# ghazalehnt/RecBole

Measured on AMD Instinct MI355X. Metric: train positives/sec (+neg) per node, higher is better.
Workload: dtype fp32; 1 GPU; C2 BPR-MF ml-20m-shape: 138,494 users x 26,745 items (incl. PAD), ~20M interactions RO_RS 0.8/0.1/0.1, embedding 128, 4 uniform negatives, 512 positives (2,048 rows) per step, dense Adam; global_batch=512, per_gpu_batch=512, train_interactions=16014928, parallelism=single, exchange_graph=True, sampler=walk (bit-exact)

## Files before the change

### include/mirec.h

```cpp
#ifndef MIREC_H
#define MIREC_H

#include <stddef.h>
#include <stdint.h>

#ifdef __cplusplus
extern "C" {
#endif

#define MIREC_ABI_VERSION 18

int mirec_abi_version(void);
const char* mirec_last_error(void);

size_t mirec_sample_walk_workspace_size(int64_t batch_keys, int64_t num);
int mirec_sample_walk(const int32_t* random_list, int64_t L, int64_t* pr_dev,
                      const int64_t* keys, int64_t n_keys, int64_t batch_keys,
                      int64_t n_batches, int64_t num,
                      const int64_t* used_ptr, const int32_t* used_cols,
                      const uint32_t* used_bits, int64_t n_bits,
                      int64_t n_key_space, int reject,
                      int64_t* out, int64_t out_stride, int32_t* status_dev,
                      void* ws, size_t ws_bytes, void* stream);

int mirec_sample_walk_segments(const int32_t* random_list, int64_t L, int64_t* pr_dev,
// ... 211 lines not shown
                            int32_t step_off, double beta1, double beta2, double eps,
                            double weight_decay, void* stream);
int mirec_adam_deferred_pair_f32(const mirec_adam_table* tables, const int64_t* n_max_uniq,
                                 int32_t d, const float* step_consts_dev,
                                 const int32_t* step_base_dev, int32_t step_off, double beta1,
                                 double beta2, double eps, double weight_decay, void* stream);

int mirec_adam_flush_f32(const mirec_adam_table* tables, int32_t n_tables, int32_t d,
                         const float* step_consts_dev, const int32_t* step_base_dev,
                         int32_t step_off, double beta1, double beta2, double eps,
                         double weight_decay, void* stream);
int mirec_adam_flush_rows_f32(const mirec_adam_table* tables, int32_t n_tables, int32_t d,
                              const int32_t* rows_per_wave, const float* step_consts_dev,
                              const int32_t* step_base_dev, int32_t step_off, double beta1,
                              double beta2, double eps, double weight_decay, void* stream);
int mirec_bpr_adam_step_f32(const mirec_adam_table* tables, const int64_t* n_max_uniq,
                            int32_t d, const int64_t* items, int64_t Bc, int32_t T, float gamma,
                            float grad_scale, float* loss_k, const int32_t* u_rec,
                            const int32_t* u_crec, const int32_t* i_rec, const int32_t* i_crec,
                            float* u_part, int32_t* u_join, float* i_part, int32_t* i_join,
                            const float* step_consts_dev, const int32_t* step_base_dev,
                            int32_t step_off, double beta1, double beta2, double eps,
                            double weight_decay, void* stream);
int mirec_step_records(const int64_t* user_keys, const int64_t* item_keys, int64_t n_batches,
                       int64_t Bc, int32_t T, int64_t n_users, int64_t n_items,
                       const int32_t* u_perm, const int32_t* u_uniq, const int32_t* u_seg,
                       const int32_t* u_nu, const int32_t* i_perm, const int32_t* i_uniq,
                       const int32_t* i_seg, const int32_t* i_nu, int32_t* u_rec,
                       int32_t* u_crec, int32_t* i_rec, int32_t* i_crec, int32_t* u_ahead,
                       int32_t* u_nah, int32_t* i_ahead, int32_t* i_nah, void* stream);
// ... 261 lines not shown
```

### recbole_amd/_native.py

```python
from __future__ import annotations

import ctypes
import os
from ctypes import c_double, c_float, c_int, c_int32, c_int64, c_size_t, c_void_p, c_char_p

import torch

_HERE = os.path.dirname(os.path.abspath(__file__))
LIB_PATH = os.environ.get("MIREC_LIB", os.path.join(_HERE, "_lib", "libmirec.so"))

_P = c_void_p


class RowsRef(ctypes.Structure):
    _fields_ = [('lo', _P), ('hi', _P), ('split', c_int64)]


class SpmmEpilogue(ctypes.Structure):
    _fields_ = [('add', RowsRef), ('add_scale', c_float), ('y', RowsRef), ('acc_in', RowsRef),
                ('acc_out', RowsRef), ('acc_scale', c_float)]


class CtxField(ctypes.Structure):
    _fields_ = [('kind', c_int32), ('seq_len', c_int32), ('ids', _P), ('vals', _P),
# ... 152 lines not shown
    "mirec_adam_flat_f32": (c_int, [_P, _P, _P, c_int64, _P, _P, _P, c_double, c_double,
                                    c_double, c_double, _P]),
    "mirec_adam_multi_f32": (c_int, [ctypes.POINTER(AdamTable), c_int32, c_int32, _P, _P,
                                     c_int32, c_double, c_double, c_double, c_double, _P]),
    "mirec_adam_deferred_f32": (c_int, [ctypes.POINTER(AdamTable), c_int32, _P, c_int32, _P,
                                        _P, c_int32, c_double, c_double, c_double, c_double,
                                        _P]),
    "mirec_adam_deferred_pair_f32": (c_int, [ctypes.POINTER(AdamTable), _P, c_int32, _P, _P,
                                             c_int32, c_double, c_double, c_double, c_double,
                                             _P]),
    "mirec_adam_flush_f32": (c_int, [ctypes.POINTER(AdamTable), c_int32, c_int32, _P, _P,
                                     c_int32, c_double, c_double, c_double, c_double, _P]),
    "mirec_adam_flush_rows_f32": (c_int, [ctypes.POINTER(AdamTable), c_int32, c_int32, _P, _P,
                                          _P, c_int32, c_double, c_double, c_double, c_double,
                                          _P]),
    "mirec_bpr_adam_step_f32": (c_int, [ctypes.POINTER(AdamTable), _P, c_int32, _P, c_int64,
                                        c_int32, ctypes.c_float, ctypes.c_float, _P, _P, _P,
                                        _P, _P, _P, _P, _P, _P, _P, _P, c_int32, c_double,
                                        c_double, c_double, c_double, _P]),
    "mirec_step_record_ints": (c_int64, [c_int64]),
    "mirec_colsum_multi_f32": (c_int, [_P, _P, _P, _P, c_int32, _P]),
    "mirec_offset_keys": (c_int, [_P, _P, c_int32, c_int64, _P, _P]),
    "mirec_bpr_fwd_bwd_at_ids_f32": (c_int, [_P, c_int64, c_int32, _P, _P, _P, c_int64, c_int32,
                                             ctypes.c_float, ctypes.c_float, _P, _P, _P]),
    "mirec_chunk_group_fits": (c_int, [c_int64, c_int32, c_int64, c_int64, c_int32]),
    "mirec_chunk_group": (c_int, [_P, _P, c_int64, c_int64, c_int32, c_int64, c_int64] + [_P] * 16
                          + [_P]),
    "mirec_step_records": (c_int, [_P, _P, c_int64, c_int64, c_int32, c_int64, c_int64, _P, _P,
                                   _P, _P, _P, _P, _P, _P, _P, _P, _P, _P, _P, _P, _P, _P,
                                   _P]),
# ... 46 lines not shown
    "mirec_seq_embed_ln_drop_fwd_f32": (c_int, [_P, c_int64, _P, _P, c_int64, c_int32, c_int32,
                                                _P, _P, c_float, c_float, ctypes.c_uint64, _P,
                                                _P, _P, _P, _P, _P]),
    "mirec_seq_embed_ln_drop_bwd_f32": (c_int, [_P, c_int64, _P, _P, c_int64, c_int32, c_int32,
                                                _P, _P, _P, _P, c_float, ctypes.c_uint64, _P,
                                                _P, _P, _P, _P, _P, _P]),
    "mirec_scale_by_f32": (c_int, [_P, c_int64, _P, _P]),
    "mirec_sampled_softmax_f32": (c_int, [_P, _P, c_int64, c_int32, _P, _P, c_int64, c_int32,
                                          c_float, _P, _P, _P, _P]),
    "mirec_rank_of_pos_f32": (c_int, [_P, _P, c_int64, c_int32, _P, _P, c_int64, c_int32, _P,
                                      _P]),
    "mirec_gather_sqnorm_f32": (c_int, [_P, c_int64, c_int32, _P, c_int64, _P, _P]),
    "mirec_gather_scale_rows_f32": (c_int, [_P, c_int64, c_int32, _P, c_int64, _P, _P, _P]),
}

ABI_VERSION = 18


class NativeError(RuntimeError):
    pass


_lib = None


def lib():
    global _lib
    if _lib is not None:
        return _lib
    if not os.path.exists(LIB_PATH):
        raise NativeError(
# ... 32 lines not shown
```

### recbole_amd/csrc/adam.hip

```cpp

#include "adam_core.h"

namespace mirec {

template <int D>
__global__ __launch_bounds__(kAdamThreads) void adam_multi_kernel(
    const AdamTables tabs, const float* __restrict__ consts, const int32_t* __restrict__ step_base,
    int step_off, AdamConsts k) {
  constexpr int VPR = D / 4;
  constexpr int RPP = kAdamThreads / VPR;
  static_assert(kAdamThreads % VPR == 0, "row width");
  __shared__ int32_t slot[kAdamRows];
  __shared__ int32_t s_range[2];

  const int si = segment_of(tabs, blockIdx.x);
  const mirec_adam_table& T = tabs.t[si];
  float* __restrict__ P = T.p;
  float* __restrict__ M = T.m;
  float* __restrict__ V = T.v;
  const int32_t* __restrict__ uniq = T.uniq;

  const int64_t lo = ((int64_t)blockIdx.x - tabs.block_start[si]) * kAdamRows;
  const int64_t hi = min(T.n_rows, lo + kAdamRows);
  if (threadIdx.x < kAdamRows) slot[threadIdx.x] = -1;
// ... 145 lines not shown
    }
  }
}

template <int D>
struct FlushVec { using T = float; };
template <> struct FlushVec<128> { using T = float2; };
template <> struct FlushVec<256> { using T = float4; };

#ifndef MIREC_FLUSH_THREADS
#define MIREC_FLUSH_THREADS 64
#endif
constexpr int kFlushRowThreads = MIREC_FLUSH_THREADS;

template <int D>
__global__ __launch_bounds__(kFlushRowThreads) void adam_flush_row_kernel(
    const AdamTables tabs, const float* __restrict__ consts, const int32_t* __restrict__ step_base,
    int step_off, AdamConsts k) {
  using V = typename FlushVec<D>::T;
  constexpr int RPB = kFlushRowThreads / 64;
  const int si = segment_of(tabs, blockIdx.x);
  const mirec_adam_table& T = tabs.t[si];
  const int64_t r = ((int64_t)blockIdx.x - tabs.block_start[si]) * RPB + (threadIdx.x >> 6);
  if (r >= T.n_rows) return;
  const int target = step_base[0] + step_off;
  const int raw = __builtin_amdgcn_readfirstlane(T.last[r]);
  const int last = min(raw, target);
  const int64_t off = r * 64 + (threadIdx.x & 63);
  const bool par = T.p_alt != nullptr;
  const bool odd = par && (target & 1);
  if (last >= target) {
    if (odd && raw != kZeroState)
      reinterpret_cast<V*>(T.p)[off] = reinterpret_cast<const V*>(T.p_alt)[off];
    return;
  }
  V p = reinterpret_cast<const V*>((par && (last & 1)) ? T.p_alt : T.p)[off];
  V m = reinterpret_cast<const V*>(T.m)[off];
  V v = reinterpret_cast<const V*>(T.v)[off];
  replay<V, true>(p, m, v, last, target, consts, k);
  MIREC_WORK(10, 1);
  if (odd) reinterpret_cast<V*>(T.p_alt)[off] = p;
  reinterpret_cast<V*>(T.p)[off] = p;
  reinterpret_cast<V*>(T.m)[off] = m;
  reinterpret_cast<V*>(T.v)[off] = v;
  if ((threadIdx.x & 63) == 0) T.last[r] = target;
}

struct FlushRows {
  int32_t r[kMaxTables];
};

template <int D>
__global__ __launch_bounds__(kAdamThreads) void adam_flush_scan_kernel(
    const AdamTables tabs, const float* __restrict__ consts, const int32_t* __restrict__ step_base,
    int step_off, AdamConsts k, FlushRows rows_per_wave) {
  using V = typename FlushVec<D>::T;
  const int si = segment_of(tabs, blockIdx.x);
  const mirec_adam_table& T = tabs.t[si];
  const int R = rows_per_wave.r[si];
  const int lane = threadIdx.x & 63;
  const int64_t r0 =
      (((int64_t)blockIdx.x - tabs.block_start[si]) * (kAdamThreads / 64) + (threadIdx.x >> 6)) * R;
  if (r0 >= T.n_rows) return;
  const int target = step_base[0] + step_off;
  const bool par = T.p_alt != nullptr;
  const bool odd = par && (target & 1);
  int raw = kZeroState;
  if (lane < R && r0 + lane < T.n_rows) raw = T.last[r0 + lane];
  const bool need = min(raw, target) < target || (odd && raw != kZeroState);
  uint64_t todo = __ballot(need);
  while (todo) {
    const int i = __builtin_ctzll(todo);
    todo &= todo - 1;
    const int64_t r = r0 + i;
    const int rraw = __shfl(raw, i, 64);
    const int last = min(rraw, target);
    const int64_t off = r * 64 + lane;
    if (last >= target) {
      reinterpret_cast<V*>(T.p)[off] = reinterpret_cast<const V*>(T.p_alt)[off];
      continue;
    }
    V p = reinterpret_cast<const V*>((par && (last & 1)) ? T.p_alt : T.p)[off];
    V m = reinterpret_cast<const V*>(T.m)[off];
    V v = reinterpret_cast<const V*>(T.v)[off];
    replay<V, true>(p, m, v, last, target, consts, k);
    MIREC_WORK(10, 1);
    if (odd) reinterpret_cast<V*>(T.p_alt)[off] = p;
    reinterpret_cast<V*>(T.p)[off] = p;
    reinterpret_cast<V*>(T.m)[off] = m;
    reinterpret_cast<V*>(T.v)[off] = v;
    if (lane == 0) T.last[r] = target;
  }
}

}

using namespace mirec;

namespace {

enum class Sched { kStreamed, kDeferred, kFlush, kDeferredPair };

int launch_adam(Sched sched, const mirec_adam_table* tables, int32_t n_tables,
                const int64_t* n_max_uniq, int32_t d, const float* consts,
                const int32_t* step_base, int32_t step_off, double beta1, double beta2,
                double eps, double weight_decay, void* stream, const char* what,
                const int32_t* flush_rows = nullptr) {
  if (n_tables < 1 || n_tables > kMaxTables || !tables || !consts || !step_base) {
    set_error("%s: bad arguments (n_tables=%d)", what, n_tables);
    return -1;
  }
  if (((uintptr_t)consts & 15) != 0) {
    set_error("%s: step constants must be 16-byte aligned", what);
    return -1;
  }
  if (d != 4 && d != 16 && d != 32 && d != 64 && d != 128 && d != 256 &&
      !(d == 1 && sched != Sched::kStreamed)) {
    set_error("%s: row width %d not in {4,16,32,64,128,256} (1: deferred / flush)", what, d);
    return -1;
  }
  const int VPR = d / 4;
  const bool pair = sched == Sched::kDeferredPair;
// ... 10 lines not shown
  for (int q = 0; q < kMaxTables; ++q) fr.r[q] = 1;
  if (sched == Sched::kFlush && flush_rows) {
    if (d < 64) {
      set_error("%s: rows per wave need d >= 64", what);
      return -1;
    }
    for (int q = 0; q < n_tables; ++q) {
      if (flush_rows[q] < 1 || flush_rows[q] > 64) {
        set_error("%s: rows per wave %d of table %d not in [1, 64]", what, flush_rows[q], q);
        return -1;
      }
      fr.r[q] = flush_rows[q];
    }
    scan = true;
  }
  AdamTables tabs;
  memset(&tabs, 0, sizeof(tabs));
  const bool deferred = sched == Sched::kDeferred;
  tabs.n_seg = deferred ? 2 * n_tables : n_tables;
  int dvec = 1;
  if (deferred && n_max_uniq && d >= 4) {
    int64_t waves = 0;
    for (int q = 0; q < (pair ? 1 : n_tables); ++q)
      if (n_max_uniq[q] > 0)
        waves += n_max_uniq[q] * (tables[q].ahead_uniq ? 2 : 1) * ((d + 63) / 64);
    if (waves > 16 * 1024) dvec = 2;
    bool ahead = false;
    for (int q = 0; q < n_tables; ++q) ahead = ahead || tables[q].ahead_uniq != nullptr;
    if (dvec == 2 && d >= 128 && !ahead && !pair) dvec = 4;
  }
// ... 3 lines not shown
    const bool grouped = t.n_uniq != nullptr;
    if (!t.p || !t.m || !t.v || t.n_rows < 0 ||
        (grouped && (!t.uniq || !t.seg || !t.perm || !t.rows)) ||
        (sched != Sched::kStreamed && !t.last) ||
        (deferred && (!grouped || t.dense_grad || !n_max_uniq || n_max_uniq[q] < 0)) ||
        (deferred && (t.ahead_uniq == nullptr) != (t.ahead_n_uniq == nullptr))) {
      set_error("%s: bad table %d", what, q);
      return -1;
    }
    if (t.p_alt && (sched == Sched::kStreamed || d < 64 || pair)) {
      set_error("%s: table %d: parity buffer (p_alt) needs the deferred schedule and d >= 64",
                what, q);
      return -1;
    }
    tabs.t[q] = t;
    if (deferred) {
      const int rpb = (pair && q == 1) ? deferred_block(1) : deferred_block(d / dvec) / (d / dvec);
      const int64_t nb = (n_max_uniq[q] + rpb - 1) / rpb;
      tabs.block_start[2 * q] = blocks;
      blocks += nb;
      tabs.block_start[2 * q + 1] = blocks;
      if (t.ahead_uniq) blocks += nb;
    } else {
      tabs.block_start[q] = blocks;
      const int64_t rows_per_block =
          scan ? (int64_t)(kAdamThreads / 64) * fr.r[q]
          : (sched == Sched::kFlush && d >= 64) ? kFlushRowThreads / 64
          : sched == Sched::kFlush ? kFlushRows
                                   : kAdamRows;
      blocks += (t.n_rows + rows_per_block - 1) / rows_per_block;
    }
// ... 15 lines not shown
  case DD:                                                                                   \
    if (sched == Sched::kStreamed)                                                           \
      hipLaunchKernelGGL(adam_multi_kernel<DD>, grd, blk, 0, st, tabs, consts, step_base,    \
                         step_off, k);                                                       \
    else if (deferred && pair)                                                               \
      hipLaunchKernelGGL((dvec == 2 ? adam_deferred_pair_kernel<DD, float2>                  \
                                    : adam_deferred_pair_kernel<DD, float>),                 \
                         grd, dim3(deferred_block(1)), 0, st, tabs, consts, step_base,       \
                         step_off, k);                                                       \
    else if (deferred)                                                                       \
      hipLaunchKernelGGL((dvec == 4 ? adam_deferred_kernel<DD, float4>                       \
                          : dvec == 2 ? adam_deferred_kernel<DD, float2>                     \
                                      : adam_deferred_kernel<DD, float>),                    \
                         grd, dim3(deferred_block(DD / dvec)), 0, st, tabs, consts,          \
                         step_base, step_off, k);                                            \
    else if (DD >= 64 && scan)                                                               \
      hipLaunchKernelGGL(adam_flush_scan_kernel<(DD >= 64 ? DD : 64)>, grd, blk, 0, st, tabs,  \
                         consts, step_base, step_off, k, fr);                                \
    else if (DD >= 64)                                                                       \
      hipLaunchKernelGGL(adam_flush_row_kernel<(DD >= 64 ? DD : 64)>, grd,                   \
                         dim3(kFlushRowThreads), 0, st, tabs,                                \
                         consts, step_base, step_off, k);                                    \
    else                                                                                     \
      hipLaunchKernelGGL(adam_flush_list_kernel<(DD < 64 ? DD : 16)>, grd, blk, 0, st, tabs, \
                         consts, step_base, step_off, k);                                    \
    break;
  switch (d) {
    case 1:
      if (deferred)
        hipLaunchKernelGGL((adam_deferred_kernel<1, float>), grd, dim3(deferred_block(1)), 0, st,
                           tabs, consts, step_base, step_off, k);
      else
        hipLaunchKernelGGL(adam_flush_list_kernel<1>, grd, blk, 0, st, tabs, consts, step_base,
// ... 66 lines not shown
extern "C" int mirec_adam_flush_rows_f32(const mirec_adam_table* tables, int32_t n_tables,
                                         int32_t d, const int32_t* rows_per_wave,
                                         const float* step_consts_dev,
                                         const int32_t* step_base_dev, int32_t step_off,
                                         double beta1, double beta2, double eps,
                                         double weight_decay, void* stream) {
  if (!rows_per_wave) {
    set_error("mirec_adam_flush_rows_f32: rows_per_wave is NULL");
    return -1;
  }
  return launch_adam(Sched::kFlush, tables, n_tables, nullptr, d, step_consts_dev,
                     step_base_dev, step_off, beta1, beta2, eps, weight_decay, stream,
                     "mirec_adam_flush_rows_f32", rows_per_wave);
}

extern "C" int mirec_adam_sparse_grad_f32(float* p, float* m, float* v, int64_t n_rows,
                                          int32_t d, const float* rows, const int32_t* perm,
                                          const int32_t* uniq, const int32_t* seg,
                                          const int32_t* n_uniq_dev, int64_t n_max_uniq,
                                          const float* dense_grad, const float* step_consts_dev,
                                          const int32_t* step_idx_dev, double beta1,
                                          double beta2, double eps, double weight_decay,
                                          void* stream) {
  (void)n_max_uniq;
  if (n_rows == 0) return 0;
  mirec_adam_table t;
  memset(&t, 0, sizeof(t));
  t.p = p; t.m = m; t.v = v; t.n_rows = n_rows;
  t.rows = rows; t.perm = perm; t.uniq = uniq; t.seg = seg; t.n_uniq = n_uniq_dev;
  t.dense_grad = dense_grad;
// ... 152 lines not shown
```

### recbole_amd/csrc/step.hip

```cpp
#include "adam_core.h"
#include "bpr_math.h"
#include "ahead.h"

namespace mirec {

struct StepLaunch {
  mirec_adam_table t[2];
  const int32_t* rec[2];
  const int32_t* crec[2];
  float* part[2];
  int32_t* join[2];
  int64_t block_start[7];
  int32_t seg_rows[6];
};

__device__ __forceinline__ int64_t clamp_id(int64_t id, int64_t n) {
  return id < 0 ? 0 : (id >= n ? n - 1 : id);
}


constexpr int kRecInts = 8;
constexpr int kRecInline = 2;
constexpr int kRowRec = 4 + kRecInline * kRecInts;
constexpr int kShare = kRecInline;
// ... 359 lines not shown
}

template <int D> struct StepVec { using T = float2; };
template <> struct StepVec<64> { using T = float; };
#ifndef MIREC_STEP_RPB
#define MIREC_STEP_RPB 4
#endif
template <int D> struct StepRows { static constexpr int n = D <= 128 ? MIREC_STEP_RPB : 1; };
#ifndef MIREC_STEP_SUM_LOADS
#define MIREC_STEP_SUM_LOADS 8
#endif
constexpr int kSumLoads = MIREC_STEP_SUM_LOADS;
#ifndef MIREC_STEP_WAVES
#define MIREC_STEP_WAVES 5
#endif

template <int D>
__global__ __launch_bounds__(D / Lanes<typename StepVec<D>::T>::n * StepRows<D>::n,
                             MIREC_STEP_WAVES)
void bpr_adam_step_kernel(
    const StepLaunch L, const int64_t* __restrict__ items, int Bc, int T, float gamma,
    float grad_scale, float* __restrict__ loss_k, const float* __restrict__ consts,
    const int32_t* __restrict__ step_base, int step_off, AdamConsts k) {
  using V = typename StepVec<D>::T;
  constexpr int EPT = Lanes<V>::n;
  constexpr int TPB = D / EPT;
  constexpr int RPB = StepRows<D>::n;
  static_assert(RPB == 1 || TPB == 64, "several rows per workgroup need one wave per row");
  constexpr int LPR = D / 4;
  constexpr int NG = TPB / LPR;
  __shared__ float cont_all[RPB][NG][D];
  __shared__ int s_last_all[RPB];
  const int wv = RPB > 1 ? __builtin_amdgcn_readfirstlane((int)(threadIdx.x / TPB)) : 0;
  auto& cont = cont_all[wv];
  int& s_last = s_last_all[wv];
  auto row_sync = [&]() {
    if (RPB == 1) {
      __syncthreads();
    } else {
      __builtin_amdgcn_fence(__ATOMIC_RELEASE, "wavefront");
      __builtin_amdgcn_wave_barrier();
      __builtin_amdgcn_fence(__ATOMIC_ACQUIRE, "wavefront");
    }
  };
  int si = 0;
// ... 250 lines not shown
    return -1;
  }
  if (n_batches == 0 || Bc == 0) return 0;
  const RecJob U = {u_perm, u_uniq, u_seg, u_nu, u_rec, u_crec, u_ahead, u_nah};
  const RecJob I = {i_perm, i_uniq, i_seg, i_nu, i_rec, i_crec, i_ahead, i_nah};
  const int64_t KI = (1 + T) * Bc;
  const int PC = (int)((KI + kPrepThreads - 1) / kPrepThreads);
  hipLaunchKernelGGL(step_prep_kernel, dim3((unsigned)(4 * n_batches + 2 * n_batches * PC)),
                     dim3(kPrepThreads), 0, (hipStream_t)stream, user_keys, item_keys,
                     (int)n_batches, (int)Bc, T, n_users, n_items, U, I, PC);
  return launch_status("mirec_step_records");
}

extern "C" int64_t mirec_step_record_ints(int64_t per) { return per < 0 ? -1 : rec_ints(per); }

#if defined(MIREC_STEP_COUNT)
extern "C" int mirec_work_counters(unsigned long long* dst, int clear) {
  if (hipMemcpyFromSymbol(dst, HIP_SYMBOL(g_work), sizeof(g_work)) != hipSuccess) return -1;
  if (clear) {
    unsigned long long z[16] = {0};
    if (hipMemcpyToSymbol(HIP_SYMBOL(g_work), z, sizeof(z)) != hipSuccess) return -1;
  }
  return 0;
}
#endif

namespace mirec {
static int bits_for(int64_t n) {
  int b = 0;
  while (b < 40 && ((int64_t)1 << b) < n) ++b;
// ... 133 lines not shown
```

### recbole_amd/trainer/chunk_plan.py

```python
from __future__ import annotations

import bisect
import math


def plan_chunks(n, Bg, C, ramp, cuts=(), ramps=(0,)):
    full = n // Bg
    bounds = sorted({0, full} | {int(c) for c in cuts if 0 < int(c) < full})
    ramp_at = {int(r) for r in ramps}
    out = []
    for lo, hi in zip(bounds[:-1], bounds[1:]):
        ri = 0 if lo in ramp_at else len(ramp)
        b0 = lo
        while b0 < hi:
            size = ramp[ri] if ri < len(ramp) else C
            ri += 1
            nb = min(size, C, hi - b0)
            out.append((b0, nb, Bg))
            b0 += nb
    if n % Bg:
        out.append((full, 1, n % Bg))
    return out


# ... 14 lines not shown
    flags, since = [], 0
    for i, (b0, nb, _) in enumerate(plan):
        entry = since > 0
        since += nb
        nxt_full = i + 1 < len(plan) and plan[i + 1][2] == Bg
        nxt_nb = plan[i + 1][1] if i + 1 < len(plan) else 0
        flush = (since >= flush_every or since + nxt_nb > flush_every * 3 // 2
                 or not nxt_full or b0 + nb in flush_at)
        if flush:
            since = 0
        flags.append((entry, flush_rows(b0 + nb, Bg, times, adam_mode, d, n_rows, busy0,
                                        max_rows) if flush else False))
    return flags


def chunk_of(plan, b):
    return max(bisect.bisect_right(plan, (b, math.inf)) - 1, 0)
```

### recbole_amd/trainer/fused.py

```python
from __future__ import annotations

import ctypes
import math
import os
from types import SimpleNamespace

import numpy as np
import torch

from recbole_amd import ops
from recbole_amd._native import AdamTable, ChunkPrep, check, lib
from recbole_amd.trainer import chunk_plan
from recbole_amd.trainer.exchange import ExchangeLayout

REC_CONTRIB = 8
ADAM_MODES = ('deferred', 'streamed')


_PREP_STREAMS = {}


def _prep_streams_for(dev, n=2):
    key = (str(dev), n)
    got = _PREP_STREAMS.get(key)
# ... 39 lines not shown


class _Slot(object):

    def __init__(self, C, B, T, G, dev, ahead, tab=None):
        Bg = G * B
        KI = (1 + T) * Bg
        self.user_keys = torch.empty(C * Bg, dtype=torch.int64, device=dev)
        self.item_keys = torch.empty(C * KI, dtype=torch.int64, device=dev)
        self.lu = self.li = None
        if G > 1:
            self.lu = torch.empty(C * B, dtype=torch.int64, device=dev)
            self.li = torch.empty(C * (1 + T) * B, dtype=torch.int64, device=dev)
        self.tab = tab or [_Lists(C, per, dev, ahead) for per in (Bg, KI)]
        self.records = None
        self.prep = None
        self.ready, self.walked, self.free = (torch.cuda.Event() for _ in range(3))
        cur = torch.cuda.current_stream(dev)
        for ev in (self.ready, self.walked, self.free):
            ev.record(cur)
        self.free_recorded = False
        self.group_pending = False
        self.ready_on_model = False
        self.chunk = None
        self.graphs = {}


class FusedBPRTrainStep(object):

    CHUNK = 64
    SLOTS = 3
    RAMP = (8, 16, 32)
    FLUSH_EVERY = 64
    FLUSH_SPARSE_MAX_ROWS = 8
    MAIN_FIRST = os.environ.get('MIREC_MAIN_FIRST', '1') != '0'
    SPEC_WALK = os.environ.get('MIREC_SPEC_WALK', '1') != '0'

    def __init__(self, model, optimizer, train_data, chunk=None, use_graph=True,
                 adam_mode='deferred', dist=None, fused_step=None):
        if adam_mode not in ADAM_MODES:
            raise ValueError(f'adam_mode must be one of {ADAM_MODES}, got {adam_mode!r}')
        self.model = model
        self.opt = optimizer
        self.data = train_data
        (self.pU, self.nU), (self.pI, self.nI) = model.fused_embedding_tables()
        self.device = self.pU.device
        self.B = train_data.step
        self.times = train_data.times
        self.uid_field = train_data.uid_field
        self.iid_field = train_data.iid_field
        self.C = chunk or self.CHUNK
# ... 9 lines not shown
            self.G, self.rank = 1, 0
        B, T, G, d = self.B, self.times, self.G, self.pU.shape[1]
        self.Bg = G * B
        self.d = d
        dev = self.device
        deferred = adam_mode == 'deferred'
        applies = deferred and G == 1 and d in (64, 128, 256)
        if fused_step and not applies:
            raise ValueError('fused_step needs adam_mode="deferred", one rank and d in '
                             '{64, 128, 256}')
        self.fused_step = applies if fused_step is None else bool(fused_step)
        self.loss_k = torch.empty(self.C * self.Bg, dtype=torch.float32, device=dev)
        self.samp_ws = torch.empty(lib().mirec_sample_walk_workspace_size(self.Bg, T),
                                   dtype=torch.uint8, device=dev)
        self.sort_ws = None
        self.prep_stream, self.group_stream = _prep_streams_for(dev)
        self.zero_i32 = torch.zeros(1, dtype=torch.int32, device=dev)
        self.loss_hist = torch.zeros(1, dtype=torch.float32, device=dev)
        self.consts = torch.zeros(4, dtype=torch.float32, device=dev)
        self.step_idx = torch.zeros(1, dtype=torch.int32, device=dev)
        self.ticket = torch.zeros(1, dtype=torch.int32, device=dev)
        self.kernel_events = None
        self.kernel_uniq = []
        self.n_eager_steps = 0
        self._rec_w = {}
        self._spec_buf = self._spec_stats = None
        self._gs_R = self._gs = None
        self._users = self._items = None
        self.n_batches = 0
        self._plan, self._flags, self._flush_at = [], [], set()
        self._busy0 = None
        self._batches_enqueued = 0
        self._current = True
        self._next_chunk = self._next_group = self._prep_limit = 0
        self._cur = None
        self._last_walked = None
        self._deferred_waits = []
        self._urgent = False
        self._late_top_up = None
        self.opt._ensure_state(self.pU)
        self.opt._ensure_state(self.pI)
        self._tables = (AdamTable * 2)()
        g = self.opt.param_groups[0]
        self._adam_args = (g['betas'][0], g['betas'][1], g['eps'], g['weight_decay'])
        self._allocate()
# ... 4 lines not shown
        self.layout = ExchangeLayout(G, B, T, d)
        self.xbuf = torch.empty(self.Bg * (2 + T) * d, dtype=torch.float32, device=dev)
        self.xchg = torch.empty(G * self.layout.W, dtype=torch.float32, device=dev)
        self.slots = [_Slot(self.C, B, T, G, dev, deferred) for _ in range(self.SLOTS)]
        self.lastU = self.lastI = None
        if deferred:
            self.lastU = torch.zeros(self.nU, dtype=torch.int32, device=dev)
            self.lastI = torch.zeros(self.nI, dtype=torch.int32, device=dev)
        self.pU_alt = torch.empty_like(self.pU.data) if self.fused_step else None
        self.pI_alt = torch.empty_like(self.pI.data) if self.fused_step else None
        self._step_scratch = None
        if self.fused_step:
            for sl in self.slots:
                sl.records = [torch.empty(self.C * w, dtype=torch.int32, device=dev)
                              for w in self._rec_ints(self.Bg)]
            self._step_scratch = ops.step_scratch(self.Bg, T, d, dev)
        self._n_max = (ctypes.c_int64 * 2)(self.Bg, (1 + T) * self.Bg)
        self._fill_tables()

    def _flush_rows(self, b_end):
        return chunk_plan.flush_rows(b_end, self.Bg, self.times, self.adam_mode, self.d,
                                     [t.n_rows for t in self._tables], self._busy0,
                                     self.FLUSH_SPARSE_MAX_ROWS)

    def _chunk_of(self, b):
        return chunk_plan.chunk_of(self._plan, b)

    def _dp_slice(self, Bc):
        return self.G > 1 and Bc == self.Bg

    def _prepare(self, slot, chunk, on=None):
        if slot.free_recorded and on is None and not slot.free.query():
            self.prep_stream.wait_event(slot.free)
        if self._dp_slice(chunk[2]):
            self._prepare_dp(slot, chunk)
        else:
            self._prepare_native(slot, chunk, on)

    def _prepare_native(self, slot, chunk, on):
        b0, nb, Bc = chunk
        cp = self._chunk_prep(slot)
        cp.users, cp.items = self._users.data_ptr(), self._items.data_ptr()
        cp.s0, cp.n_batches, cp.Bc = b0 * self.Bg, nb, Bc
        samp = self.data.sampler
        if samp.alias is not None:
            thr, idx, cp.alias_seed, cp.alias_counter = samp.alias_args(
                self.device, nb * Bc * self.times)
            cp.alias_thr, cp.alias_idx, cp.n_alias = thr.data_ptr(), idx.data_ptr(), thr.numel()
# ... 52 lines not shown
        slot.chunk = chunk

    def _apply_deferred_waits(self):
        for st, ev in self._deferred_waits:
            st.wait_event(ev)
        self._deferred_waits = []

    def _prepare_group(self, slot):
        self._apply_deferred_waits()
        self.group_stream.wait_event(slot.walked)
        self._group_on(slot, self.group_stream)

    def _group_on(self, slot, st):
        check(lib().mirec_prepare_chunk_group(ctypes.byref(slot.prep), st.cuda_stream),
              'mirec_prepare_chunk_group')
        slot.ready.record(st)
        slot.group_pending = False

    def _chunk_prep(self, slot):
        if slot.prep is not None:
            return slot.prep
        dev = self.device
        with torch.cuda.stream(self.prep_stream):
            walk = self.data.sampler.walk_args(dev)
        rl, pr, up, uc, bits, n_bits, reject, status = walk
        T = self.times
        nsort = lib().mirec_segment_sort_workspace_size(self.C * (1 + T) * self.Bg, self.nI)
        if self.sort_ws is None or self.sort_ws.numel() < nsort:
            self.sort_ws = torch.empty(nsort, dtype=torch.uint8, device=dev)
        p = lambda x: x.data_ptr() if x is not None else None
# ... 158 lines not shown
                                      n_steps, float(Bc * self.times),
                                      self.loss_hist.data_ptr(), self.step_idx.data_ptr(),
                                      self.ticket.data_ptr(), stream.cuda_stream)
        check(rc, 'mirec_chunk_finish')

    def _flush(self, stream, rows=None):
        if self.adam_mode != 'deferred':
            return
        if rows is not None and any(r > 1 for r in rows):
            self._launch('flush', stream, 'mirec_adam_flush_rows_f32', self._tables, 2, self.d,
                         (ctypes.c_int32 * 2)(*rows), *self._sched(0))
        else:
            self._launch('flush', stream, 'mirec_adam_flush_f32', self._tables, 2, self.d,
                         *self._sched(0))

    def _entry_lists(self, slot):
        return [(l.uniq, l.nu) for l in slot.tab]

    def _entry(self, slot, stream):
        if self.adam_mode != 'deferred':
            return
        t = (AdamTable * 2)()
        ctypes.memmove(t, self._tables, ctypes.sizeof(t))
        self._point_tables(t, [SimpleNamespace(perm=uniq, uniq=uniq, seg=uniq, nu=self.zero_i32,
                                               ahead=uniq, nah=n)
                               for uniq, n in self._entry_lists(slot)], 0, (0, 0), True)
        t[0].rows = t[1].rows = self.xbuf.data_ptr()
        self._adam(stream, -1, t, 'ahead')

    def _grad_scale(self, Bc):
        R = Bc * self.times
        if self._gs_R != R:
            self._gs_R = R
            self._gs = float(np.float32(1.0) / np.float32(R))
        return self._gs

    def _graph_for(self, slot, nb, entry, flush):
        key = (nb, entry, flush)
        g = slot.graphs.get(key)
        if g is None:
            g = torch.cuda.CUDAGraph()
            cap = torch.cuda.Stream(device=self.device)
            cap.wait_stream(torch.cuda.current_stream(self.device))
            with torch.cuda.graph(g, stream=cap):
                if entry:
                    self._entry(slot, cap)
                for c in range(nb):
                    self._step(slot, c, self.Bg, cap, c, c + 1 < nb)
                self._finish(0, nb, self.Bg, cap)
                if flush:
                    self._flush(cap, flush)
            torch.cuda.current_stream(self.device).wait_stream(cap)
            slot.graphs[key] = g
        return g

    def _capture_variants(self):
        S = len(self.slots)
        variants = sorted({(k % S, n, e, f) for k, ((_, n, Bc), (e, f)) in
                           enumerate(zip(self._plan, self._flags)) if Bc == self.Bg},
                          key=lambda v: (v[0], v[1], v[2], repr(v[3])))
        for k, n, e, f in variants:
            self._graph_for(self.slots[k], n, e, f)

    def begin_epoch(self, cuts=(), hold_prep_from=None, flush_at=()):
        data = self.data
        if data.shuffle:
            data._shuffle()
        inter = data.dataset.inter_feat
        self._users = inter[self.uid_field]
        self._items = inter[self.iid_field]
        if not self._users.is_cuda:
            raise RuntimeError('fused train step needs the train table on the GPU')
        self.n_batches = nb = math.ceil(self._users.numel() / self.Bg)
        table = self.opt.step_constants(self.opt.n_steps + 1, max(nb, 1)).reshape(-1)
        ptrs = [(t.p, t.m, t.v) for t in self._tables]
        self._fill_tables()
        stale = ptrs != [(t.p, t.m, t.v) for t in self._tables]
        if self.consts.numel() < table.size:
            self.consts = torch.zeros(table.size, dtype=torch.float32, device=self.device)
# ... 11 lines not shown
            busy = []
            for m, v, last in self._adam_state():
                ops.zero_state_marks(m, v, last, self._adam_args[3])
                busy.append((last != ops.ADAM_ZERO_STATE).sum())
            self._busy0 = [int(x) for x in torch.stack(busy).cpu()]
        if self.fused_step:
            self.pU_alt.copy_(self.pU.data)
            self.pI_alt.copy_(self.pI.data)
        ramps = (0,) if hold_prep_from is None else (0, int(hold_prep_from))
        self._plan = chunk_plan.plan_chunks(self._users.numel(), self.Bg, self.C, self.RAMP,
                                            cuts, ramps)
        self._flush_at = set(int(b) for b in flush_at)
        self._flags = chunk_plan.chunk_flags(self._plan, self.Bg, self.FLUSH_EVERY,
                                             self._flush_at, self.times, self.adam_mode, self.d,
                                             n_rows, self._busy0, self.FLUSH_SPARSE_MAX_ROWS)
        if self.use_graph:
            self._capture_variants()
        self.prep_stream.wait_stream(torch.cuda.current_stream(self.device))
        self._last_walked = None
        self._deferred_waits, self._urgent, self._late_top_up = [], False, None
        self._next_chunk = 0
        self._next_group = 0
        self._prep_limit = (len(self._plan) if hold_prep_from is None
                            else self._chunk_of(hold_prep_from))
        self._cur = None
        for s in self.slots:
            s.free_recorded = False
            if not self._dp_slice(self.Bg):
                self._chunk_prep(s)
        for _ in range(len(self.slots)):
# ... 49 lines not shown
        self._issue_groups(k + 1)
        slot = self.slots[k % S]
        if self._late_top_up != k:
            self._top_up_prep(k)
        if not slot.ready_on_model:
            stream.wait_event(slot.ready)
        self._cur = k

    def run_batches(self, b_start, b_end):
        stream = torch.cuda.current_stream(self.device)
        b = b_start
        while b < b_end:
            k = self._chunk_of(b)
            b0, nb, Bc = self._plan[k]
            entry, flush = self._flags[k]
            self._enter_chunk(k, stream)
            slot = self.slots[k % len(self.slots)]
            c0, c1 = b - b0, min(nb, b_end - b0)
            key = (nb, entry, flush)
            if (self.use_graph and c0 == 0 and c1 == nb and Bc == self.Bg
                    and self.kernel_events is None and key in slot.graphs):
                slot.graphs[key].replay()
                self._current = flush
            else:
                self.n_eager_steps += c1 - c0
                if c0 == 0 and entry:
                    self._entry(slot, stream)
                for c in range(c0, c1):
                    self._step(slot, c, Bc, stream, 0, c + 1 < nb)
                    self._finish(c, 1, Bc, stream)
                self._current = False
                if c1 == nb and flush:
                    self._flush(stream, flush)
                    self._current = True
            if self._late_top_up == k:
                self._late_top_up = None
                self._urgent = True
                self._top_up_prep(k)
                self._urgent = False
            self._issue_groups(k + len(self.slots))
            b = b0 + c1
            self._batches_enqueued = b

    def _top_up_prep(self, k):
        lim = min(len(self._plan), self._prep_limit, k + len(self.slots))
        while self._next_chunk < lim:
            self._issue_prep()

    def sync_params(self):
        if not self._current:
            self._flush(torch.cuda.current_stream(self.device),
                        self._flush_rows(self._batches_enqueued))
            self._current = True

    def end_epoch(self, n_done=None):
        n_done = self.n_batches if n_done is None else n_done
        stream = torch.cuda.current_stream(self.device)
        stream.wait_stream(self.prep_stream)
        stream.wait_stream(self.group_stream)
        self.sync_params()
        self.opt.advance(n_done)
        self.data.pr = 0
        self.data.sampler.check_status()
        return [float(x) for x in self.loss_hist[:n_done].cpu().numpy()]

    def run_epoch(self):
        nb = self.begin_epoch()
        self.run_batches(0, nb)
        return self.end_epoch()

    def close(self):
        torch.cuda.synchronize(self.device)
        self._drop_graphs()
        torch.cuda.synchronize(self.device)

    def _drop_graphs(self):
        for s in self.slots:
            s.graphs = {}


from recbole_amd.trainer.fused_eval import (fused_full_sort_eval,
                                            fused_general_sampled_eval,
                                            fused_seq_full_sort_eval, fused_seq_sampled_eval)
from recbole_amd.trainer.sharded import ShardedBPRTrainStep
```

Measured before the change: 25.48 million positives/s.

## Overlap deferred Adam flush of untouched user rows on a background stream

Splits the periodic deferred-Adam flush into two parts. A per-chunk bitmap marks the user rows the chunk touches. Rows the chunk does not touch are flushed by a new persistent walk kernel on a separate background stream while the chunk's graph runs, and only the touched rows plus the items are flushed inside the graph. The fused step kernel also raises its wave priority with s_setprio so the background flush does not slow it. This adds a bitmap build per chunk, extra graph variants, and cross-stream event waits, and the two streams contend for bandwidth and CUs.

```diff
diff --git a/include/mirec.h b/include/mirec.h
--- a/include/mirec.h
+++ b/include/mirec.h
@@ -8,7 +8,7 @@
 extern "C" {
 #endif
 
-#define MIREC_ABI_VERSION 18
+#define MIREC_ABI_VERSION 19
 
 int mirec_abi_version(void);
 const char* mirec_last_error(void);
@@ -250,6 +250,14 @@
                               const int32_t* rows_per_wave, const float* step_consts_dev,
                               const int32_t* step_base_dev, int32_t step_off, double beta1,
                               double beta2, double eps, double weight_decay, void* stream);
+int mirec_adam_flush_masked_f32(const mirec_adam_table* tables, int32_t n_tables, int32_t d,
+                                const uint32_t* const* masks, const int32_t* want,
+                                const int32_t* rows_per_wave, int32_t walk_waves,
+                                const float* step_consts_dev, const int32_t* step_base_dev,
+                                int32_t step_off, double beta1, double beta2, double eps,
+                                double weight_decay, void* stream);
+int mirec_row_bitmap(const int64_t* keys, int64_t n_keys, int64_t n_rows, uint32_t* bitmap,
+                     void* stream);
 int mirec_bpr_adam_step_f32(const mirec_adam_table* tables, const int64_t* n_max_uniq,
                             int32_t d, const int64_t* items, int64_t Bc, int32_t T, float gamma,
                             float grad_scale, float* loss_k, const int32_t* u_rec,
diff --git a/recbole_amd/_native.py b/recbole_amd/_native.py
--- a/recbole_amd/_native.py
+++ b/recbole_amd/_native.py
@@ -190,6 +190,10 @@
     "mirec_adam_flush_rows_f32": (c_int, [ctypes.POINTER(AdamTable), c_int32, c_int32, _P, _P,
                                           _P, c_int32, c_double, c_double, c_double, c_double,
                                           _P]),
+    "mirec_adam_flush_masked_f32": (c_int, [ctypes.POINTER(AdamTable), c_int32, c_int32, _P, _P,
+                                            _P, c_int32, _P, _P, c_int32, c_double, c_double,
+                                            c_double, c_double, _P]),
+    "mirec_row_bitmap": (c_int, [_P, c_int64, c_int64, _P, _P]),
     "mirec_bpr_adam_step_f32": (c_int, [ctypes.POINTER(AdamTable), _P, c_int32, _P, c_int64,
                                         c_int32, ctypes.c_float, ctypes.c_float, _P, _P, _P,
                                         _P, _P, _P, _P, _P, _P, _P, _P, c_int32, c_double,
@@ -266,7 +270,7 @@
     "mirec_gather_scale_rows_f32": (c_int, [_P, c_int64, c_int32, _P, c_int64, _P, _P, _P]),
 }
 
-ABI_VERSION = 18
+ABI_VERSION = 19
 
 
 class NativeError(RuntimeError):
diff --git a/recbole_amd/csrc/adam.hip b/recbole_amd/csrc/adam.hip
--- a/recbole_amd/csrc/adam.hip
+++ b/recbole_amd/csrc/adam.hip
@@ -183,19 +183,13 @@
 constexpr int kFlushRowThreads = MIREC_FLUSH_THREADS;
 
 template <int D>
-__global__ __launch_bounds__(kFlushRowThreads) void adam_flush_row_kernel(
-    const AdamTables tabs, const float* __restrict__ consts, const int32_t* __restrict__ step_base,
-    int step_off, AdamConsts k) {
+__device__ __forceinline__ void flush_row(const mirec_adam_table& T, int64_t r, int raw,
+                                          int target, int lane,
+                                          const float* __restrict__ consts,
+                                          const AdamConsts& k) {
   using V = typename FlushVec<D>::T;
-  constexpr int RPB = kFlushRowThreads / 64;
-  const int si = segment_of(tabs, blockIdx.x);
-  const mirec_adam_table& T = tabs.t[si];
-  const int64_t r = ((int64_t)blockIdx.x - tabs.block_start[si]) * RPB + (threadIdx.x >> 6);
-  if (r >= T.n_rows) return;
-  const int target = step_base[0] + step_off;
-  const int raw = __builtin_amdgcn_readfirstlane(T.last[r]);
   const int last = min(raw, target);
-  const int64_t off = r * 64 + (threadIdx.x & 63);
+  const int64_t off = r * 64 + lane;
   const bool par = T.p_alt != nullptr;
   const bool odd = par && (target & 1);
   if (last >= target) {
@@ -212,18 +206,44 @@
   reinterpret_cast<V*>(T.p)[off] = p;
   reinterpret_cast<V*>(T.m)[off] = m;
   reinterpret_cast<V*>(T.v)[off] = v;
-  if ((threadIdx.x & 63) == 0) T.last[r] = target;
+  if (lane == 0) T.last[r] = target;
+}
+
+__device__ __forceinline__ bool flush_needs(const mirec_adam_table& T, int raw, int target) {
+  return min(raw, target) < target || (T.p_alt != nullptr && (target & 1) && raw != kZeroState);
+}
+
+template <int D>
+__global__ __launch_bounds__(kFlushRowThreads) void adam_flush_row_kernel(
+    const AdamTables tabs, const float* __restrict__ consts, const int32_t* __restrict__ step_base,
+    int step_off, AdamConsts k) {
+  constexpr int RPB = kFlushRowThreads / 64;
+  const int si = segment_of(tabs, blockIdx.x);
+  const mirec_adam_table& T = tabs.t[si];
+  const int64_t r = ((int64_t)blockIdx.x - tabs.block_start[si]) * RPB + (threadIdx.x >> 6);
+  if (r >= T.n_rows) return;
+  const int target = step_base[0] + step_off;
+  const int raw = __builtin_amdgcn_readfirstlane(T.last[r]);
+  flush_row<D>(T, r, raw, target, threadIdx.x & 63, consts, k);
 }
 
 struct FlushRows {
   int32_t r[kMaxTables];
 };
-
-template <int D>
+struct FlushMasks {
+  const uint32_t* bits[kMaxTables];
+  int32_t want[kMaxTables];
+};
+
+__device__ __forceinline__ bool mask_selects(const uint32_t* __restrict__ bits, int want,
+                                             int64_t r) {
+  return !bits || (int)((bits[r >> 5] >> (r & 31)) & 1u) == want;
+}
+
+template <int D, bool MASKED>
 __global__ __launch_bounds__(kAdamThreads) void adam_flush_scan_kernel(
     const AdamTables tabs, const float* __restrict__ consts, const int32_t* __restrict__ step_base,
-    int step_off, AdamConsts k, FlushRows rows_per_wave) {
-  using V = typename FlushVec<D>::T;
+    int step_off, AdamConsts k, FlushRows rows_per_wave, FlushMasks masks) {
   const int si = segment_of(tabs, blockIdx.x);
   const mirec_adam_table& T = tabs.t[si];
   const int R = rows_per_wave.r[si];
@@ -232,33 +252,44 @@
       (((int64_t)blockIdx.x - tabs.block_start[si]) * (kAdamThreads / 64) + (threadIdx.x >> 6)) * R;
   if (r0 >= T.n_rows) return;
   const int target = step_base[0] + step_off;
-  const bool par = T.p_alt != nullptr;
-  const bool odd = par && (target & 1);
   int raw = kZeroState;
-  if (lane < R && r0 + lane < T.n_rows) raw = T.last[r0 + lane];
-  const bool need = min(raw, target) < target || (odd && raw != kZeroState);
-  uint64_t todo = __ballot(need);
+  if (lane < R && r0 + lane < T.n_rows &&
+      (!MASKED || mask_selects(masks.bits[si], masks.want[si], r0 + lane)))
+    raw = T.last[r0 + lane];
+  uint64_t todo = __ballot(flush_needs(T, raw, target));
   while (todo) {
     const int i = __builtin_ctzll(todo);
     todo &= todo - 1;
-    const int64_t r = r0 + i;
-    const int rraw = __shfl(raw, i, 64);
-    const int last = min(rraw, target);
-    const int64_t off = r * 64 + lane;
-    if (last >= target) {
-      reinterpret_cast<V*>(T.p)[off] = reinterpret_cast<const V*>(T.p_alt)[off];
-      continue;
-    }
-    V p = reinterpret_cast<const V*>((par && (last & 1)) ? T.p_alt : T.p)[off];
-    V m = reinterpret_cast<const V*>(T.m)[off];
-    V v = reinterpret_cast<const V*>(T.v)[off];
-    replay<V, true>(p, m, v, last, target, consts, k);
-    MIREC_WORK(10, 1);
-    if (odd) reinterpret_cast<V*>(T.p_alt)[off] = p;
-    reinterpret_cast<V*>(T.p)[off] = p;
-    reinterpret_cast<V*>(T.m)[off] = m;
-    reinterpret_cast<V*>(T.v)[off] = v;
-    if (lane == 0) T.last[r] = target;
+    flush_row<D>(T, r0 + i, __shfl(raw, i, 64), target, lane, consts, k);
+  }
+}
+
+constexpr int kWalkRows = 32;
+
+template <int D>
+__global__ __launch_bounds__(64) void adam_flush_walk_kernel(
+    const AdamTables tabs, const float* __restrict__ consts, const int32_t* __restrict__ step_base,
+    int step_off, AdamConsts k, FlushMasks masks) {
+  const int lane = threadIdx.x;
+  const int target = step_base[0] + step_off;
+  for (int si = 0; si < tabs.n_seg; ++si) {
+    const mirec_adam_table& T = tabs.t[si];
+    const uint32_t* __restrict__ bits = masks.bits[si];
+    const uint32_t flip = masks.want[si] ? 0u : ~0u;
+    const int64_t groups = (T.n_rows + kWalkRows - 1) / kWalkRows;
+    for (int64_t g = blockIdx.x; g < groups; g += gridDim.x) {
+      const int64_t r0 = g * kWalkRows;
+      const uint32_t sel = bits ? (bits[g] ^ flip) : ~0u;
+      int raw = kZeroState;
+      if (lane < kWalkRows && r0 + lane < T.n_rows && ((sel >> lane) & 1u))
+        raw = T.last[r0 + lane];
+      uint64_t todo = __ballot(flush_needs(T, raw, target));
+      while (todo) {
+        const int i = __builtin_ctzll(todo);
+        todo &= todo - 1;
+        flush_row<D>(T, r0 + i, __shfl(raw, i, 64), target, lane, consts, k);
+      }
+    }
   }
 }
 
@@ -274,7 +305,8 @@
                 const int64_t* n_max_uniq, int32_t d, const float* consts,
                 const int32_t* step_base, int32_t step_off, double beta1, double beta2,
                 double eps, double weight_decay, void* stream, const char* what,
-                const int32_t* flush_rows = nullptr) {
+                const int32_t* flush_rows = nullptr, const FlushMasks* masks = nullptr,
+                int walk_waves = 0) {
   if (n_tables < 1 || n_tables > kMaxTables || !tables || !consts || !step_base) {
     set_error("%s: bad arguments (n_tables=%d)", what, n_tables);
     return -1;
@@ -315,6 +347,14 @@
     }
     scan = true;
   }
+  const bool walk = masks && walk_waves > 0;
+  if (masks && (sched != Sched::kFlush || d < 64 || (!scan && !walk))) {
+    set_error("%s: a masked flush needs d >= 64 and rows per wave or a wave count", what);
+    return -1;
+  }
+  FlushMasks fm;
+  memset(&fm, 0, sizeof(fm));
+  if (masks) fm = *masks;
   AdamTables tabs;
   memset(&tabs, 0, sizeof(tabs));
   const bool deferred = sched == Sched::kDeferred;
@@ -348,7 +388,10 @@
       return -1;
     }
     tabs.t[q] = t;
-    if (deferred) {
+    if (walk) {
+      tabs.block_start[q] = 0;
+      if (t.n_rows > 0) blocks = walk_waves;
+    } else if (deferred) {
       const int rpb = (pair && q == 1) ? deferred_block(1) : deferred_block(d / dvec) / (d / dvec);
       const int64_t nb = (n_max_uniq[q] + rpb - 1) / rpb;
       tabs.block_start[2 * q] = blocks;
@@ -394,9 +437,15 @@
                                       : adam_deferred_kernel<DD, float>),                    \
                          grd, dim3(deferred_block(DD / dvec)), 0, st, tabs, consts,          \
                          step_base, step_off, k);                                            \
+    else if (DD >= 64 && walk)                                                               \
+      hipLaunchKernelGGL(adam_flush_walk_kernel<(DD >= 64 ? DD : 64)>, grd, dim3(64), 0, st,   \
+                         tabs, consts, step_base, step_off, k, fm);                          \
+    else if (DD >= 64 && scan && masks)                                                      \
+      hipLaunchKernelGGL((adam_flush_scan_kernel<(DD >= 64 ? DD : 64), true>), grd, blk, 0,    \
+                         st, tabs, consts, step_base, step_off, k, fr, fm);                  \
     else if (DD >= 64 && scan)                                                               \
-      hipLaunchKernelGGL(adam_flush_scan_kernel<(DD >= 64 ? DD : 64)>, grd, blk, 0, st, tabs,  \
-                         consts, step_base, step_off, k, fr);                                \
+      hipLaunchKernelGGL((adam_flush_scan_kernel<(DD >= 64 ? DD : 64), false>), grd, blk, 0,   \
+                         st, tabs, consts, step_base, step_off, k, fr, fm);                  \
     else if (DD >= 64)                                                                       \
       hipLaunchKernelGGL(adam_flush_row_kernel<(DD >= 64 ? DD : 64)>, grd,                   \
                          dim3(kFlushRowThreads), 0, st, tabs,                                \
@@ -493,6 +542,43 @@
                      "mirec_adam_flush_rows_f32", rows_per_wave);
 }
 
+extern "C" int mirec_adam_flush_masked_f32(const mirec_adam_table* tables, int32_t n_tables,
+                                           int32_t d, const uint32_t* const* masks,
+                                           const int32_t* want, const int32_t* rows_per_wave,
+                                           int32_t walk_waves, const float* step_consts_dev,
+                                           const int32_t* step_base_dev, int32_t step_off,
+                                           double beta1, double beta2, double eps,
+                                           double weight_decay, void* stream) {
+  const char* what = "mirec_adam_flush_masked_f32";
+  if (!tables || n_tables < 1 || n_tables > kMaxTables || !want || walk_waves < 0 ||
+      walk_waves > 65536 || (walk_waves == 0) != (rows_per_wave != nullptr)) {
+    set_error("%s: bad arguments (rows per wave for the scan form, or a wave count in "
+              "[1, 65536] for the walk form)", what);
+    return -1;
+  }
+  mirec_adam_table sel[kMaxTables];
+  int32_t rows[kMaxTables];
+  FlushMasks fm;
+  memset(&fm, 0, sizeof(fm));
+  int n = 0;
+  for (int q = 0; q < n_tables; ++q) {
+    if (want[q] < 0) continue;
+    if (want[q] > 1) {
+      set_error("%s: want[%d] = %d not in {-1, 0, 1}", what, q, want[q]);
+      return -1;
+    }
+    sel[n] = tables[q];
+    rows[n] = rows_per_wave ? rows_per_wave[q] : 1;
+    fm.bits[n] = masks ? masks[q] : nullptr;
+    fm.want[n] = want[q];
+    ++n;
+  }
+  if (n == 0) return 0;
+  return launch_adam(Sched::kFlush, sel, n, nullptr, d, step_consts_dev, step_base_dev, step_off,
+                     beta1, beta2, eps, weight_decay, stream, what,
+                     rows_per_wave ? rows : nullptr, &fm, walk_waves);
+}
+
 extern "C" int mirec_adam_sparse_grad_f32(float* p, float* m, float* v, int64_t n_rows,
                                           int32_t d, const float* rows, const int32_t* perm,
                                           const int32_t* uniq, const int32_t* seg,
diff --git a/recbole_amd/csrc/step.hip b/recbole_amd/csrc/step.hip
--- a/recbole_amd/csrc/step.hip
+++ b/recbole_amd/csrc/step.hip
@@ -397,6 +397,9 @@
 #ifndef MIREC_STEP_WAVES
 #define MIREC_STEP_WAVES 5
 #endif
+#ifndef MIREC_STEP_PRIO
+#define MIREC_STEP_PRIO 3
+#endif
 
 template <int D>
 __global__ __launch_bounds__(D / Lanes<typename StepVec<D>::T>::n * StepRows<D>::n,
@@ -412,6 +415,7 @@
   static_assert(RPB == 1 || TPB == 64, "several rows per workgroup need one wave per row");
   constexpr int LPR = D / 4;
   constexpr int NG = TPB / LPR;
+  __builtin_amdgcn_s_setprio(MIREC_STEP_PRIO);
   __shared__ float cont_all[RPB][NG][D];
   __shared__ int s_last_all[RPB];
   const int wv = RPB > 1 ? __builtin_amdgcn_readfirstlane((int)(threadIdx.x / TPB)) : 0;
@@ -692,6 +696,34 @@
 
 extern "C" int64_t mirec_step_record_ints(int64_t per) { return per < 0 ? -1 : rec_ints(per); }
 
+namespace mirec {
+__global__ __launch_bounds__(256) void row_bitmap_kernel(const int64_t* __restrict__ keys,
+                                                         int64_t n_keys, int64_t n_rows,
+                                                         uint32_t* __restrict__ bitmap) {
+  const int64_t i = (int64_t)blockIdx.x * blockDim.x + threadIdx.x;
+  if (i >= n_keys) return;
+  const int64_t r = clamp_id(keys[i], n_rows);
+  atomicOr(bitmap + (r >> 5), 1u << (r & 31));
+}
+}
+
+extern "C" int mirec_row_bitmap(const int64_t* keys, int64_t n_keys, int64_t n_rows,
+                                uint32_t* bitmap, void* stream) {
+  const char* what = "mirec_row_bitmap";
+  if (n_keys < 0 || n_rows <= 0 || !bitmap || (n_keys > 0 && !keys) ||
+      n_keys > (int64_t)INT32_MAX * 256) {
+    set_error("%s: bad arguments", what);
+    return -1;
+  }
+  hipStream_t st = (hipStream_t)stream;
+  const int rc = hip_status(hipMemsetAsync(bitmap, 0, (size_t)((n_rows + 31) / 32) * 4, st), what);
+  if (rc) return rc;
+  if (n_keys == 0) return 0;
+  hipLaunchKernelGGL(row_bitmap_kernel, dim3((unsigned)((n_keys + 255) / 256)), dim3(256), 0, st,
+                     keys, n_keys, n_rows, bitmap);
+  return launch_status(what);
+}
+
 #if defined(MIREC_STEP_COUNT)
 extern "C" int mirec_work_counters(unsigned long long* dst, int clear) {
   if (hipMemcpyFromSymbol(dst, HIP_SYMBOL(g_work), sizeof(g_work)) != hipSuccess) return -1;
diff --git a/recbole_amd/trainer/chunk_plan.py b/recbole_amd/trainer/chunk_plan.py
--- a/recbole_amd/trainer/chunk_plan.py
+++ b/recbole_amd/trainer/chunk_plan.py
@@ -52,5 +52,24 @@
     return flags
 
 
+def bg_flush_chunks(plan, flags, Bg, adam_mode, fused_step, use_graph, min_steps=1,
+                    enabled=True):
+    on = bool(enabled and fused_step and use_graph and adam_mode == 'deferred')
+    return [bool(on and flush and not entry and Bc == Bg and nb >= min_steps)
+            for (_, nb, Bc), (entry, flush) in zip(plan, flags)]
+
+
+def bg_flush_now(planned, c0, c1, nb, graph_ready, timed_kernels):
+    return bool(planned and c0 == 0 and c1 == nb and graph_ready and not timed_kernels)
+
+
+def masked_flush_rows(flush, nb, Bg, n_users, max_rows):
+    frac = min(1.0, nb * Bg / max(n_users, 1))
+    r = 1
+    while r * 2 <= max_rows and r * 2 * frac <= 1.0:
+        r *= 2
+    return (r,) + tuple(flush[1:])
+
+
 def chunk_of(plan, b):
     return max(bisect.bisect_right(plan, (b, math.inf)) - 1, 0)
diff --git a/recbole_amd/trainer/fused.py b/recbole_amd/trainer/fused.py
--- a/recbole_amd/trainer/fused.py
+++ b/recbole_amd/trainer/fused.py
@@ -77,6 +77,9 @@
             self.li = torch.empty(C * (1 + T) * B, dtype=torch.int64, device=dev)
         self.tab = tab or [_Lists(C, per, dev, ahead) for per in (Bg, KI)]
         self.records = None
+        self.bitmap = None
+        self.bg_done = None
+        self.bg_busy = False
         self.prep = None
         self.ready, self.walked, self.free = (torch.cuda.Event() for _ in range(3))
         cur = torch.cuda.current_stream(dev)
@@ -98,6 +101,9 @@
     FLUSH_SPARSE_MAX_ROWS = 8
     MAIN_FIRST = os.environ.get('MIREC_MAIN_FIRST', '1') != '0'
     SPEC_WALK = os.environ.get('MIREC_SPEC_WALK', '1') != '0'
+    BG_FLUSH = os.environ.get('MIREC_BG_FLUSH', '1') != '0'
+    BG_WAVES = int(os.environ.get('MIREC_BG_WAVES', '1536'))
+    BG_MIN_STEPS = 32
 
     def __init__(self, model, optimizer, train_data, chunk=None, use_graph=True,
                  adam_mode='deferred', dist=None, fused_step=None):
@@ -137,7 +143,9 @@
         self.samp_ws = torch.empty(lib().mirec_sample_walk_workspace_size(self.Bg, T),
                                    dtype=torch.uint8, device=dev)
         self.sort_ws = None
-        self.prep_stream, self.group_stream = _prep_streams_for(dev)
+        side = _prep_streams_for(dev, 3 if self.fused_step else 2)
+        self.prep_stream, self.group_stream = side[:2]
+        self.bg_stream = side[2] if self.fused_step else None
         self.zero_i32 = torch.zeros(1, dtype=torch.int32, device=dev)
         self.loss_hist = torch.zeros(1, dtype=torch.float32, device=dev)
         self.consts = torch.zeros(4, dtype=torch.float32, device=dev)
@@ -152,6 +160,10 @@
         self._users = self._items = None
         self.n_batches = 0
         self._plan, self._flags, self._flush_at = [], [], set()
+        self._bg = []
+        self._bg_pending = None
+        self._bg_mark = torch.cuda.Event()
+        self._bg_mark.record(torch.cuda.current_stream(dev))
         self._busy0 = None
         self._batches_enqueued = 0
         self._current = True
@@ -186,6 +198,9 @@
             for sl in self.slots:
                 sl.records = [torch.empty(self.C * w, dtype=torch.int32, device=dev)
                               for w in self._rec_ints(self.Bg)]
+                sl.bitmap = torch.zeros((self.nU + 31) // 32, dtype=torch.int32, device=dev)
+                sl.bg_done = torch.cuda.Event()
+                sl.bg_done.record(torch.cuda.current_stream(dev))
             self._step_scratch = ops.step_scratch(self.Bg, T, d, dev)
         self._n_max = (ctypes.c_int64 * 2)(self.Bg, (1 + T) * self.Bg)
         self._fill_tables()
@@ -204,6 +219,9 @@
     def _prepare(self, slot, chunk, on=None):
         if slot.free_recorded and on is None and not slot.free.query():
             self.prep_stream.wait_event(slot.free)
+        if slot.bg_busy:
+            (on if on is not None else self.prep_stream).wait_event(slot.bg_done)
+            slot.bg_busy = False
         if self._dp_slice(chunk[2]):
             self._prepare_dp(slot, chunk)
         else:
@@ -286,6 +304,11 @@
     def _group_on(self, slot, st):
         check(lib().mirec_prepare_chunk_group(ctypes.byref(slot.prep), st.cuda_stream),
               'mirec_prepare_chunk_group')
+        b0, nb, Bc = slot.chunk
+        if slot.bitmap is not None and self._bg[self._chunk_of(b0)]:
+            check(lib().mirec_row_bitmap(slot.user_keys.data_ptr(), nb * Bc, self.nU,
+                                         slot.bitmap.data_ptr(), st.cuda_stream),
+                  'mirec_row_bitmap')
         slot.ready.record(st)
         slot.group_pending = False
 
@@ -474,6 +497,31 @@
             self._launch('flush', stream, 'mirec_adam_flush_f32', self._tables, 2, self.d,
                          *self._sched(0))
 
+    def _flush_masked(self, stream, slot, rows):
+        self._launch('flush', stream, 'mirec_adam_flush_masked_f32', self._tables, 2, self.d,
+                     (ctypes.c_void_p * 2)(slot.bitmap.data_ptr(), None),
+                     (ctypes.c_int32 * 2)(1, 1), (ctypes.c_int32 * 2)(*rows), 0,
+                     *self._sched(0))
+
+    def _flush_background(self, slot, t_end, stream):
+        bg = self.bg_stream
+        self._bg_mark.record(stream)
+        bg.wait_event(self._bg_mark)
+        bg.wait_event(slot.ready)
+        check(lib().mirec_adam_flush_masked_f32(
+            self._tables, 2, self.d, (ctypes.c_void_p * 2)(slot.bitmap.data_ptr(), None),
+            (ctypes.c_int32 * 2)(0, -1), None, int(self.BG_WAVES), self.consts.data_ptr(),
+            self.zero_i32.data_ptr(), int(t_end), *self._adam_args, bg.cuda_stream),
+            'mirec_adam_flush_masked_f32')
+        slot.bg_done.record(bg)
+        slot.bg_busy = True
+        self._bg_pending = slot.bg_done
+
+    def _await_background(self, stream):
+        if self._bg_pending is not None:
+            stream.wait_event(self._bg_pending)
+            self._bg_pending = None
+
     def _entry_lists(self, slot):
         return [(l.uniq, l.nu) for l in slot.tab]
 
@@ -495,8 +543,8 @@
             self._gs = float(np.float32(1.0) / np.float32(R))
         return self._gs
 
-    def _graph_for(self, slot, nb, entry, flush):
-        key = (nb, entry, flush)
+    def _graph_for(self, slot, nb, entry, flush, masked=False):
+        key = (nb, entry, flush, masked)
         g = slot.graphs.get(key)
         if g is None:
             g = torch.cuda.CUDAGraph()
@@ -508,7 +556,10 @@
                 for c in range(nb):
                     self._step(slot, c, self.Bg, cap, c, c + 1 < nb)
                 self._finish(0, nb, self.Bg, cap)
-                if flush:
+                if flush and masked:
+                    self._flush_masked(cap, slot, chunk_plan.masked_flush_rows(
+                        flush, nb, self.Bg, self.nU, self.FLUSH_SPARSE_MAX_ROWS))
+                elif flush:
                     self._flush(cap, flush)
             torch.cuda.current_stream(self.device).wait_stream(cap)
             slot.graphs[key] = g
@@ -516,13 +567,14 @@
 
     def _capture_variants(self):
         S = len(self.slots)
-        variants = sorted({(k % S, n, e, f) for k, ((_, n, Bc), (e, f)) in
-                           enumerate(zip(self._plan, self._flags)) if Bc == self.Bg},
-                          key=lambda v: (v[0], v[1], v[2], repr(v[3])))
-        for k, n, e, f in variants:
-            self._graph_for(self.slots[k], n, e, f)
+        variants = sorted({(k % S, n, e, f, bg) for k, ((_, n, Bc), (e, f), bg) in
+                           enumerate(zip(self._plan, self._flags, self._bg)) if Bc == self.Bg},
+                          key=lambda v: (v[0], v[1], v[2], repr(v[3]), v[4]))
+        for k, n, e, f, bg in variants:
+            self._graph_for(self.slots[k], n, e, f, bg)
 
     def begin_epoch(self, cuts=(), hold_prep_from=None, flush_at=()):
+        self._await_background(torch.cuda.current_stream(self.device))
         data = self.data
         if data.shuffle:
             data._shuffle()
@@ -564,6 +616,9 @@
         self._flags = chunk_plan.chunk_flags(self._plan, self.Bg, self.FLUSH_EVERY,
                                              self._flush_at, self.times, self.adam_mode, self.d,
                                              n_rows, self._busy0, self.FLUSH_SPARSE_MAX_ROWS)
+        self._bg = chunk_plan.bg_flush_chunks(self._plan, self._flags, self.Bg, self.adam_mode,
+                                              self.fused_step, self.use_graph,
+                                              self.BG_MIN_STEPS, self.BG_FLUSH)
         if self.use_graph:
             self._capture_variants()
         self.prep_stream.wait_stream(torch.cuda.current_stream(self.device))
@@ -643,12 +698,16 @@
             k = self._chunk_of(b)
             b0, nb, Bc = self._plan[k]
             entry, flush = self._flags[k]
+            self._await_background(stream)
             self._enter_chunk(k, stream)
             slot = self.slots[k % len(self.slots)]
             c0, c1 = b - b0, min(nb, b_end - b0)
-            key = (nb, entry, flush)
+            key = (nb, entry, flush, self._bg[k])
             if (self.use_graph and c0 == 0 and c1 == nb and Bc == self.Bg
                     and self.kernel_events is None and key in slot.graphs):
+                if chunk_plan.bg_flush_now(self._bg[k], c0, c1, nb, key in slot.graphs,
+                                           self.kernel_events is not None):
+                    self._flush_background(slot, b0 + nb, stream)
                 slot.graphs[key].replay()
                 self._current = flush
             else:
@@ -677,6 +736,7 @@
             self._issue_prep()
 
     def sync_params(self):
+        self._await_background(torch.cuda.current_stream(self.device))
         if not self._current:
             self._flush(torch.cuda.current_stream(self.device),
                         self._flush_rows(self._batches_enqueued))
@@ -685,6 +745,7 @@
     def end_epoch(self, n_done=None):
         n_done = self.n_batches if n_done is None else n_done
         stream = torch.cuda.current_stream(self.device)
+        self._await_background(stream)
         stream.wait_stream(self.prep_stream)
         stream.wait_stream(self.group_stream)
         self.sync_params()
@@ -699,6 +760,7 @@
         return self.end_epoch()
 
     def close(self):
+        self._await_background(torch.cuda.current_stream(self.device))
         torch.cuda.synchronize(self.device)
         self._drop_graphs()
         torch.cuda.synchronize(self.device)
```

New measurement: 26.67 million positives/s, median of 6. 1.05x the previous value.
